# nlamprian/ICP

Measured on AMD Instinct MI355X. Metric: ICP iterations/sec at |F|=|M|=16384, |R|=256, higher is better.
Workload: dtype f32

## Files before the change

### icp_amd/csrc/icp_capi.hip

```cpp
#include "icp_host.h"

using namespace icp_host;

namespace {

void free_all (icp_context *h)
{
    drop_graphs (h);
    for (void *q : h->dev_allocs) (void) hipFree (q);
    h->dev_allocs.clear ();
    if (h->hF) (void) hipHostFree (h->hF);
    if (h->hM) (void) hipHostFree (h->hM);
    if (h->hT) (void) hipHostFree (h->hT);
    if (h->hState) (void) hipHostFree (h->hState);
    if (h->hMirror) (void) hipHostFree (h->hMirror);
    if (h->hTrackMirror) (void) hipHostFree (h->hTrackMirror);
    h->hState = nullptr; h->hMirror = h->hTrackMirror = nullptr; h->hstate_fresh = false;
    h->run = run_ctl {}; h->track_k_hist[0] = h->track_k_hist[1] = 0; h->track_hist_frame = 0;
    if (h->dCloud) (void) hipFree (h->dCloud);
    if (h->dCloudOut) (void) hipFree (h->dCloudOut);
    h->hF = h->hM = h->hT = nullptr; h->dCloud = h->dCloudOut = nullptr; h->cloud_cap = 0;
    h->dF = h->dM = nullptr; h->ownF = h->ownM = true;
    for (int k = 0; k < 2; ++k) {
        if (h->hBand[k]) (void) hipHostFree (h->hBand[k]);
// ... 132 lines not shown
    if (h->stream2) (void) hipStreamDestroy (h->stream2);
    if (h->stream) (void) hipStreamDestroy (h->stream);
    delete h;
    return ICP_OK;
}
ICP_CATCH_ALL

static int write_color_kappa (icp_context *h)
{
    uint32_t bits; std::memcpy (&bits, &h->color_kappa, sizeof bits);
    HIPCHK (h, hipMemsetD32Async (reinterpret_cast<hipDeviceptr_t> (icp_color_kappa (h->p)), (int) bits, 1, h->stream));
    return ICP_OK;
}

static int write_robust_scale (icp_context *h)
{
    uint32_t bits; std::memcpy (&bits, &h->robust_scale, sizeof bits);
    HIPCHK (h, hipMemsetD32Async (reinterpret_cast<hipDeviceptr_t> (icp_robust_scale (h->p)), (int) bits, 1, h->stream));
    return ICP_OK;
}

int icp_init_batched (icp_handle h, uint32_t batch, uint32_t m, uint32_t nr, float a, float c,
                      uint32_t max_iterations, double angle_threshold, double translation_threshold) try
{
    api_guard guard_ (h);
    if (!h) return ICP_EINVAL;
    if (m == 0) return fail (h, ICP_EINVAL, "The sets of landmarks cannot have zero points");
    if (nr == 0) return fail (h, ICP_EINVAL, "The sets of representatives cannot have zero points");
    if (a == 0.f) return fail (h, ICP_EINVAL, "The alpha parameter cannot be equal to zero");
    if (m % 2) return fail (h, ICP_EINVAL, "The number of points in the array must be a multiple of 2");
    if (batch == 0 || batch > 65535u) return fail (h, ICP_EINVAL, "batch must be in [1, 65535]");
    if (max_iterations == 0) return fail (h, ICP_EINVAL, "max_iterations must be positive");
    uint32_t nrx, nry, side;
    if (!reps_grid (m, nr, &nrx, &nry, &side))
        return fail (h, ICP_EINVAL, "nr must be a power of two whose grid tiles the sqrt(m) x sqrt(m) landmark grid");
    if (nr > 32768u) return fail (h, ICP_EINVAL, "nr must be <= 32768");
    if (m > (1u << 20)) return fail (h, ICP_EINVAL, "m must be <= 2^20");
    int rc = set_device (h); if (rc) return rc;
    if ((rc = run_close_all (h))) return rc;
    if (h->copy_stream) HIPCHK (h, hipStreamSynchronize (h->copy_stream));
    if (h->stream2) HIPCHK (h, hipStreamSynchronize (h->stream2));
    if (h->stream) HIPCHK (h, hipStreamSynchronize (h->stream));
    int rot = h->p.rot, weighted = h->p.weighted, pmode = h->p.power_mode, fused = h->p.fused, chain = h->p.chain;
    const float dist_scale = h->p.dist_scale;
    const uint32_t reject = h->p.reject; const float reject_d2 = h->p.reject_d2, reject_max_dist = h->p.reject_max_dist, trim_keep = h->p.trim_keep;
    const uint32_t metric = h->p.metric, nrm_grid = h->p.nrm_grid; const float p2pl_mu = h->p.p2pl_mu;
    free_all (h);
    icp_params &p = h->p;
    p = icp_params {};
    p.rot = rot; p.weighted = weighted; p.power_mode = pmode; p.check = 0; p.fused = fused; p.chain = chain; p.emit = 1;
    p.dist_scale = dist_scale;
    p.reject = reject; p.reject_d2 = reject_d2; p.reject_max_dist = reject_max_dist; p.trim_keep = trim_keep;
    p.metric = metric; p.nrm_grid = nrm_grid; p.p2pl_mu = p2pl_mu;
    p.m = m; p.nr = nr; p.batch = batch; p.side = side; p.nrx = nrx; p.nry = nry;
    p.a = a; p.c = c;
    {
        auto magic = [] (uint32_t d) { return d > 1u ? (uint32_t) ((1ull << 32) / d + 1ull) : 0u; };
        p.side_magic = magic (side); p.cellw_magic = magic (side / nrx); p.cellh_magic = magic (side / nry);
    }
    h->max_iterations = max_iterations; h->angle_threshold = angle_threshold; h->translation_threshold = translation_threshold;
    p.tan_half_thr = std::tan (angle_threshold * M_PI / 360.0);
    p.trans_thr = translation_threshold;
    p.nwg = (m + 127u) / 128u;
    p.nwp = p.nwg; if (p.nwp != 1 && (p.nwp % 4)) p.nwp += 4 - p.nwp % 4;
    uint32_t n4 = m; if (n4 % 4) n4 += 4 - n4 % 4;
    p.G = n4 / 4;
    p.nsp = (p.G + 511u) / 512u; if (p.nsp != 1 && (p.nsp % 4)) p.nsp += 4 - p.nsp % 4;
    p.nchunk = (m + ICP_CHUNK - 1) / ICP_CHUNK;
    p.nb = (m + 63u) / 64u;
    { const uint32_t ng = (p.nb + 127u) / 128u; p.ng_magic = ng > 1u ? (uint32_t) ((1ull << 32) / ng + 1ull) : 0u; }

    const size_t B = batch;
    float *F = nullptr, *M = nullptr;
    if ((rc = dalloc (h, &F, B * m * 8))) return rc;
    if ((rc = dalloc (h, &M, B * m * 8))) return rc;
    h->dF = F; h->dM = M; p.F = F; p.M = M; h->lm[0] = F; h->lm[1] = M;
    if ((rc = dalloc (h, &p.R, B * nr * 8))) return rc;
    p.n16 = (nr + 15u) / 16u;
    p.nb = (m + 63u) / 64u;
    p.tbox = icp_tbox_of (p); p.n1k = (nr + p.tbox - 1u) / p.tbox;
    p.s2wave = icp_s2_wave_of (p);
    { const char *e = std::getenv ("ICP_AMD_XCDMAP"); p.xcdmap = e ? (e[0] == '1') : (B == 1u); }
    { const char *e = std::getenv ("ICP_AMD_WARM_SEED"); p.warm_seed = (e && e[0] == '1') ? 1u : 0u; }
    p.gtile = 0u;
    if (nrx % 4u == 0u && nry % 4u == 0u && !std::getenv ("ICP_AMD_STRIP_GROUPS")) { uint32_t lg = 0; while ((4u << lg) < nrx) ++lg; p.gtile = lg + 1u; }
    if ((rc = dalloc (h, &p.GB, B * 2 * (p.n16 + p.n1k)))) return rc;
    if ((rc = dalloc (h, &p.XP, icp_xp_layout_of (batch, m).total))) return rc;
    if ((rc = dalloc (h, &p.XQ, B * m * 8))) return rc;
    if ((rc = dalloc (h, &p.OL, B * ICP_OL_STRIDE (nr)))) return rc;
    p.nlb = m / 16u + 2u;
    if ((rc = dalloc (h, &p.LB, B * 3 * p.nlb))) return rc;
    if ((rc = dalloc (h, &p.rep_src, B * nr))) return rc;
    if ((rc = dalloc (h, &p.owner, B * m))) return rc;
    if ((rc = dalloc (h, &p.N, 2 * B * nr))) return rc;
    if ((rc = dalloc (h, &p.O, B * nr))) return rc;
    if ((rc = dalloc (h, &p.perm, B * m))) return rc;
    if ((rc = dalloc (h, &p.chunk_hist, B * p.nchunk * nr))) return rc;
    if ((rc = dalloc (h, &p.blist, B * p.nb * 64))) return rc;
    if ((rc = dalloc (h, &p.bn, B * p.nb))) return rc;
    if ((rc = dalloc (h, &p.brank, B * m))) return rc;
    if ((rc = dalloc (h, &p.rid, B * m))) return rc;
    if ((rc = dalloc (h, &p.nn_id, B * m))) return rc;
    if ((rc = dalloc (h, &p.PF, B * m))) return rc;
    if ((rc = dalloc (h, &p.PM, B * m))) return rc;
    if ((rc = dalloc (h, &p.wpart, B * 2 * p.nwp))) return rc;
    if ((rc = dalloc (h, &p.mpart, B * 2 * p.nwg))) return rc;
    if ((rc = dalloc (h, &p.mscr, B * 2 * ((p.nwg + 127u) / 128u)))) return rc;
    if ((rc = dalloc (h, &p.spart, B * 11 * p.nsp * 8))) return rc;
    if ((rc = dalloc (h, &p.mom, icp_mom_layout_of (batch, m, p.nb).total))) return rc;
    if ((rc = write_color_kappa (h))) return rc;
    if ((rc = write_robust_scale (h))) return rc;
    if ((rc = dalloc (h, &p.ml1, B * 18 * ((p.nb + 127u) / 128u)))) return rc;
    if ((rc = dalloc (h, &p.cst, B * 2))) return rc;
    if ((rc = dalloc (h, &p.st, B))) return rc;
    if ((rc = dalloc (h, &p.st_prev, B))) return rc;
    if (!h->dTin) HIPCHK (h, hipMalloc ((void **) &h->dTin, 8 * sizeof (float)));
    HIPCHK (h, hipHostMalloc ((void **) &h->hF, B * m * 8 * sizeof (float), hipHostMallocDefault));
    HIPCHK (h, hipHostMalloc ((void **) &h->hM, B * m * 8 * sizeof (float), hipHostMallocDefault));
    HIPCHK (h, hipHostMalloc ((void **) &h->hT, 64 * sizeof (float), hipHostMallocDefault));
    HIPCHK (h, hipHostMalloc ((void **) &h->hState, B * sizeof (icp_reg_state), hipHostMallocMapped | hipHostMallocCoherent));
    HIPCHK (h, hipHostMalloc ((void **) &h->hMirror, B * sizeof (unsigned long long), hipHostMallocMapped | hipHostMallocCoherent));
    std::memset (h->hMirror, 0, B * sizeof (unsigned long long));
    icp_launch_reset_state (p, h->stream, 1);
    HIPCHK (h, hipGetLastError ());
    HIPCHK (h, hipStreamSynchronize (h->stream));
    h->inited = true; h->built = false;
    return ICP_OK;
}
ICP_CATCH_ALL

int icp_init (icp_handle h, uint32_t m, uint32_t nr, float a, float c, uint32_t max_iterations,
              double angle_threshold, double translation_threshold) try
{
    api_guard guard_ (h);
    return icp_init_batched (h, 1, m, nr, a, c, max_iterations, angle_threshold, translation_threshold);
}
ICP_CATCH_ALL

int icp_write_b (icp_handle h, uint32_t b, int mem, const void *host_ptr, int block) try
{
    api_guard guard_ (h);
    int rc = need (h, false); if (rc) return rc;
    if (b >= h->p.batch) return fail (h, ICP_EINVAL, "batch index out of range");
    if ((rc = set_device (h))) return rc;
    const size_t fm = (size_t) h->p.m * 8 * sizeof (float);
    switch (mem) {
        case ICP_MEM_F:
        case ICP_MEM_M: {
            float *stage = (mem == ICP_MEM_F ? h->hF : h->hM) + (size_t) b * h->p.m * 8;
            float *dst = (mem == ICP_MEM_F ? h->dF : h->dM) + (size_t) b * h->p.m * 8;
            hipEvent_t ev = h->evStage[mem == ICP_MEM_F ? 0 : 1];
            note_inputs_change (h);
            HIPCHK (h, hipEventSynchronize (ev));
            if (host_ptr) std::memcpy (stage, host_ptr, fm);
            HIPCHK (h, hipMemcpyAsync (dst, stage, fm, hipMemcpyHostToDevice, h->stream));
            HIPCHK (h, hipEventRecord (ev, h->stream));
            break;
        }
        case ICP_MEM_T: {
            HIPCHK (h, hipEventSynchronize (h->evStage[2]));
            if (host_ptr) std::memcpy (h->hT, host_ptr, 8 * sizeof (float));
            HIPCHK (h, hipMemcpyAsync (h->dTin, h->hT, 8 * sizeof (float), hipMemcpyHostToDevice, h->stream));
            HIPCHK (h, hipEventRecord (h->evStage[2], h->stream));
            { const long long kb = h->k_base; note_enqueue (h); h->k_base = kb; }
            icp_launch_set_T (h->p, b, h->dTin, h->stream);
            HIPCHK (h, hipGetLastError ());
// ... 860 lines not shown
```

### icp_amd/csrc/icp_search.h

```cpp
#pragma once
#include "icp_kernels.h"

static __device__ __forceinline__ float sum4 (float4 v) { return ((v.x + v.y) + v.z) + v.w; }
static __device__ __forceinline__ uint32_t ks_hole_bit (float4 mg) { return (mg.x == 0.f && mg.y == 0.f && mg.z == 0.f) ? 0x80000000u : 0u; }

#define KS_SPLIT LPQ
#define KS_QPW (64 / KS_SPLIT)
#define KS_TILE 1024u
#ifndef ICP_S2_DEPTH16
#define ICP_S2_DEPTH16 8u
#endif
#ifndef ICP_S2_UNCOND
#define ICP_S2_UNCOND 128u
#endif
#ifndef ICP_S1_ORIGIN_LIST
#define ICP_S1_ORIGIN_LIST 1
#endif
#ifndef ICP_OL_STAGED_MIN
#define ICP_OL_STAGED_MIN 32u
#endif
#ifndef ICP_S1_SEED
#define ICP_S1_SEED 1
#endif
#ifndef ICP_S1_REJECT_MIN_NR
// ... 562 lines not shown
    unsigned long long k4[4], k2[2], k1;
#pragma unroll
    for (int j = 0; j < 4; ++j) {
        const bool odd = (lane & 1u) != 0u;
        const unsigned long long keep = odd ? key[2 * j + 1] : key[2 * j], send = odd ? key[2 * j] : key[2 * j + 1];
        k4[j] = min64 (keep, xchg_dpp (send, std::integral_constant<int, 0xB1> {}));
    }
#pragma unroll
    for (int j = 0; j < 2; ++j) {
        const bool odd = (lane & 2u) != 0u;
        const unsigned long long keep = odd ? k4[2 * j + 1] : k4[2 * j], send = odd ? k4[2 * j] : k4[2 * j + 1];
        k2[j] = min64 (keep, xchg_dpp (send, std::integral_constant<int, 0x4E> {}));
    }
    {
        const bool odd = (lane & 4u) != 0u;
        const unsigned long long keep = odd ? k2[1] : k2[0], send = odd ? k2[0] : k2[1];
        k1 = min64 (keep, xchg_lane (send, lane ^ 4u));
    }
    k1 = min64 (k1, xchg_lane (k1, lane ^ 8u));
    k1 = min64 (k1, xchg_lane (k1, lane ^ 16u));
    k1 = min64 (k1, xchg_lane (k1, lane ^ 32u));
    k1 = xchg_lane (k1, (lane & 56u) | (lane >> 3));
    dmin = __uint_as_float ((uint32_t) (k1 >> 32)); jmin = (uint32_t) k1;
    {
        uint32_t nl = (je - o + 7u) >> 3;
        nl = max (nl, (uint32_t) __builtin_amdgcn_update_dpp (0, (int) nl, 0x140, 0xF, 0xF, true));
        nl = max (nl, (uint32_t) __builtin_amdgcn_update_dpp ((int) nl, (int) nl, 0x142, 0xA, 0xF, false));
        nl = max (nl, (uint32_t) __builtin_amdgcn_update_dpp ((int) nl, (int) nl, 0x143, 0xC, 0xF, false));
        const uint32_t ntrips = (uint32_t) __builtin_amdgcn_readlane ((int) nl, 63);
        if (__builtin_expect (ntrips > ICP_S2W_UNCOND / 8u, 0)) {
            const uint32_t ss = lane & 7u;
            float best2 = dmin; uint32_t bj = 0xFFFFFFFFu;
            const float4 a4 = s_qa[qe], c4 = s_qc[qe];
            ks_list_tail<8> (XQb, o, je, (max (je, 1u) - 1u) << 5, ICP_S2W_UNCOND / 16u, ntrips, a4.x, a4.y, a4.z, c4.x, c4.y, c4.z, alpha, dr, b, lane, ss, best2, bj);
            const uint32_t pos = bj != 0xFFFFFFFFu ? min (o + ss + bj * 8u, max (je, 1u) - 1u) : jmin;
            const float d2 = ks_grp_min_f<8> (best2);
            jmin = ks_grp_min_u<8> (best2 == d2 ? pos : 0xFFFFFFFFu);
            dmin = d2;
        }
    }
}

template <int LPQ>
static __device__ __forceinline__ void ks_stage2_lanes (const char *XQb, uint32_t o, uint32_t n, bool valid, float qx, float qy, float qz, float qr, float qg, float qb,
                                                        float alpha, float dr, uint32_t b, uint32_t lane, uint32_t ss, float &dmin, uint32_t &jmin)
{
    float best2 = __builtin_inff (); uint32_t bj = 0xFFFFFFFFu;
    const float2v vq_xr = { qx, qr }, vq_yg = { qy, qg }, vq_zb = { qz, qb };
    {
        constexpr uint32_t KS_DEPTH = (KS_SPLIT == 16) ? ICP_S2_DEPTH16 : 4u;
        const uint32_t je = valid ? o + n : o;
        uint32_t nl = (je - o + KS_SPLIT - 1u) / KS_SPLIT;
        if (KS_SPLIT == 8) nl = max (nl, (uint32_t) __builtin_amdgcn_update_dpp (0, (int) nl, 0x140, 0xF, 0xF, true));
        nl = max (nl, (uint32_t) __builtin_amdgcn_update_dpp ((int) nl, (int) nl, 0x142, 0xA, 0xF, false));
        nl = max (nl, (uint32_t) __builtin_amdgcn_update_dpp ((int) nl, (int) nl, 0x143, 0xC, 0xF, false));
        const uint32_t ntrips = (uint32_t) __builtin_amdgcn_readlane ((int) nl, 63);
        const uint32_t alast = (max (je, 1u) - 1u) << 5;
        constexpr uint32_t KS_UNC = ICP_S2_UNCOND / KS_SPLIT;
        const uint32_t ntr0 = (ICP_S2_UNCOND == 0u || ntrips <= 2u * KS_UNC) ? ntrips : KS_UNC;
        for (uint32_t tb = 0; tb < ntr0; tb += KS_DEPTH) {
            const uint32_t a0 = (o + ss + tb * KS_SPLIT) << 5, nt = min (KS_DEPTH, ntr0 - tb);
            float4 g[KS_DEPTH], c[KS_DEPTH];
#pragma unroll
            for (uint32_t t = 0; t < KS_DEPTH; ++t) {
                if (t >= nt) break;
                const char *rec = XQb + min (a0 + t * (KS_SPLIT * 32u), alast);
                g[t] = *reinterpret_cast<const float4 *> (rec); c[t] = *reinterpret_cast<const float4 *> (rec + 16);
            }
#pragma unroll
            for (uint32_t t = 0; t < KS_DEPTH; ++t) {
                if (t >= nt) break;
                KS_CAND (g[t], c[t], tb + t);
            }
        }
        if (__builtin_expect (ntrips > ntr0, 0))
            ks_list_tail<LPQ> (XQb, o, je, alast, ICP_S2_UNCOND / 16u, ntrips, qx, qy, qz, qr, qg, qb, alpha, dr, b, lane, ss, best2, bj);
        if (bj != 0xFFFFFFFFu) bj = min (o + ss + bj * KS_SPLIT, max (je, 1u) - 1u);
        if (je == o) { best2 = __builtin_inff (); bj = 0xFFFFFFFFu; }
    }
    dmin = ks_grp_min_f<KS_SPLIT> (best2);
    jmin = ks_grp_min_u<KS_SPLIT> (best2 == dmin ? bj : 0xFFFFFFFFu);
}

template <bool FUSED, bool CHAIN, int MINW, int LPQ, bool OWNER, bool PRUNE, bool REJ>
static __device__ __forceinline__ void ks_epilogue (const icp_params &p, float4 *s_qa, uint4 *s_qb, const float4 *s_qc, const uint32_t *s_slot, double (*s_mom)[64], float *s_w, const float4 *R4, const char *XQb,
                                                    uint32_t b, uint32_t m, uint32_t nr, uint32_t check_flags, uint32_t tid, uint32_t lane, uint32_t slice, uint32_t tile_id,
                                                    uint32_t qe, uint32_t ss, uint32_t i, bool valid, uint32_t o, uint32_t n, uint32_t rstar, float dr, float dmin, uint32_t jmin,
                                                    float qx, float qy, float qz)
{
    if (ss == 0u) {
        const bool empty = (n == 0u);
        s_qa[qe] = make_float4 (qx, qy, qz, empty ? dr : dmin);
        s_qb[qe] = make_uint4 (empty ? rstar : ((jmin == 0xFFFFFFFFu) ? o : jmin), rstar, (valid ? 1u : 0u) | (empty ? 2u : 0u), i);
    }
    __syncthreads ();
    if (slice == 0u) {
        const float4 qa = s_qa[lane]; const uint4 qb = s_qb[lane];
        const uint32_t eo = (PRUNE && ICP_S1_ORIGIN_LIST) ? s_slot[lane] : lane;
        const bool v = (qb.z & 1u) != 0u, empty = (qb.z & 2u) != 0u;
        const float ex = qa.x, ey = qa.y, ez = qa.z, d = p.dist_scale * qa.w;
        const uint32_t ei = qb.w;
        float w = 0.f, f0 = 0.f, f1 = 0.f, f2 = 0.f;
        bool acc = v;
        if (v) {
            uint32_t id;
            if (empty) {
                const float4 nn = R4[2 * (size_t) qb.x];
                const uint32_t *rsrc = p.rep_src;
                if constexpr (MINW == 4) {
                    typedef uint32_t __attribute__ ((address_space (1))) *gu32;
                    rsrc = (const uint32_t *) (gu32) ks_params_from_kernarg ()->rep_src;
                }
                id = rsrc[(size_t) b * nr + qb.x]; f0 = nn.x; f1 = nn.y; f2 = nn.z;
            } else {
                const char *rec = XQb + (qb.x << 5);
                const float4 wg = *reinterpret_cast<const float4 *> (rec), wc = *reinterpret_cast<const float4 *> (rec + 16);
                f0 = wg.x; f1 = wg.z; f2 = wc.x; id = __float_as_uint (wc.z);
            }
            w = p.weighted ? 100.f / (100.f + d) : 1.f;
            if constexpr (REJ) {
                bool rej = false;
                if (p.reject & 1u)
                    rej = (__float_as_uint (s_qc[lane].w) >> 31) != 0u || (f0 == 0.f && f1 == 0.f && f2 == 0.f);
                if (p.reject & ICP_REJECT_DIST_ON) {
                    const float gx = ex - f0, gy = ey - f1, gz = ez - f2;
                    rej = rej || !(((gx * gx + gy * gy) + gz * gz) <= p.reject_d2);
                }
                if (rej) { w = 0.f; acc = false; }
            }
            icp_dist_id di; di.dist = d; di.id = id;
            const icp_params *pe = &p;
            if constexpr (MINW == 2 && !OWNER) {
                            pe = ks_params_from_kernarg ();
            }
            typedef char __attribute__ ((address_space (1))) *gchar;
            char *o_nn = (char *) (gchar) reinterpret_cast<char *> (pe->nn_id + (size_t) b * m), *o_pf = (char *) (gchar) reinterpret_cast<char *> (pe->PF + (size_t) b * m);
            char *o_pm = (char *) (gchar) reinterpret_cast<char *> (pe->PM + (size_t) b * m), *o_rid = (char *) (gchar) reinterpret_cast<char *> (pe->rid + (size_t) b * m);
            const bool emit = !FUSED || (check_flags & 8u);
            if (emit) {
                *reinterpret_cast<icp_dist_id *> (o_nn + (ei << 3)) = di;
                *reinterpret_cast<float4 *> (o_pf + (ei << 4)) = make_float4 (f0, f1, f2, w);
                *reinterpret_cast<float4 *> (o_pm + (ei << 4)) = make_float4 (ex, ey, ez, d);
            }
            if (emit || PRUNE) *reinterpret_cast<uint32_t *> (o_rid + (ei << 2)) = qb.y;
        }
        if constexpr (FUSED) {
            double W = (double) w;
            double g0 = acc ? (double) f0 : 0.0, g1 = acc ? (double) f1 : 0.0, g2 = acc ? (double) f2 : 0.0;
            double q0 = (double) ex, q1 = (double) ey, q2 = (double) ez;
            if (!acc) { W = 0.0; q0 = q1 = q2 = 0.0; }
            double wq0 = W * q0, wq1 = W * q1, wq2 = W * q2;
            s_mom[0][eo] = W;
            s_mom[1][eo] = W * g0; s_mom[2][eo] = W * g1; s_mom[3][eo] = W * g2;
            s_mom[4][eo] = wq0; s_mom[5][eo] = wq1; s_mom[6][eo] = wq2;
            s_mom[7][eo] = wq0 * g0; s_mom[8][eo] = wq0 * g1; s_mom[9][eo] = wq0 * g2;
            s_mom[10][eo] = wq1 * g0; s_mom[11][eo] = wq1 * g1; s_mom[12][eo] = wq1 * g2;
            s_mom[13][eo] = wq2 * g0; s_mom[14][eo] = wq2 * g1; s_mom[15][eo] = wq2 * g2;
            s_mom[16][eo] = W * ((g0 * g0 + g1 * g1) + g2 * g2);
            s_mom[17][eo] = W * ((q0 * q0 + q1 * q1) + q2 * q2);
        } else
            s_w[eo] = w;
    }
    KS_STAMP (6)
    __syncthreads ();
    if constexpr (FUSED) {
        if (slice * 4u >= (uint32_t) ICP_NMOM) return;
        const uint32_t l = lane & 15u, mrow = slice * 4u + (lane >> 4);
        const uint32_t k = min (mrow, (uint32_t) ICP_NMOM - 1u);
        double c0 = s_mom[k][l] + s_mom[k][l + 32], c1 = s_mom[k][l + 16] + s_mom[k][l + 48];
        double v = row_tree_tail_d (c0 + c1);
        const uint32_t obuf = CHAIN ? (p.slot ^ 1u) : 0u;
        double *momw = p.mom;
        if constexpr (MINW == 4) {
            typedef double __attribute__ ((address_space (1))) *gf64;
            momw = (double *) (gf64) ks_params_from_kernarg ()->mom;
        }
        if (l == 0 && mrow < ICP_NMOM) momw[(((size_t) b * 2 + obuf) * ICP_NMOM + mrow) * p.nb + tile_id] = v;
    } else if (slice == 0 && (p.weighted || REJ)) {
        const uint32_t l = lane & 15u;
        float a[4] = { s_w[l], s_w[l + 16], s_w[l + 32], s_w[l + 48] };
        float v = row_tree4 (a);
        if (lane == 0) p.wpart[(size_t) b * 2 * p.nwp + blockIdx.x] = v;
    }
    KS_STAMP (7)
}

static __device__ __forceinline__ void ks_owner_lists_tail (const icp_params &p, uint4 *s_qb, uint32_t b, uint32_t m, uint32_t nb, uint32_t lane, uint32_t slice, uint32_t qe,
                                                            uint32_t ss, bool valid, uint32_t rstar)
{
    if (ss == 0u) s_qb[qe] = make_uint4 (rstar, valid ? 1u : 0u, 0u, 0u);
    __syncthreads ();
    if (slice != 0u) return;
    const uint4 e4 = s_qb[lane];
    const bool v = e4.y != 0u;
    const uint32_t own = v ? e4.x : 0xFFFFFFFFu, ip = blockIdx.x * 64u + lane;
    uint32_t rank = 0u, kk = 0u;
    uint2 *bl = p.blist + ((size_t) b * nb + blockIdx.x) * 64u;
    for (unsigned long long rem = __ballot (v); rem; ++kk) {
        const uint32_t o = (uint32_t) __builtin_amdgcn_readlane ((int) own, (int) __builtin_ctzll (rem));
        const unsigned long long same = __ballot (own == o);
        if (own == o) rank = (uint32_t) __builtin_popcountll (same & ((1ull << lane) - 1ull));
        if (lane == 0) bl[kk] = make_uint2 (o, (uint32_t) __builtin_popcountll (same));
        rem &= ~same;
    }
    if (lane == 0) p.bn[(size_t) b * nb + blockIdx.x] = kk;
    if (v) { p.owner[(size_t) b * m + ip] = own; p.brank[(size_t) b * m + ip] = (uint8_t) rank; }
    return;
}

template <int LPQ, int TILE>
static __device__ __forceinline__ uint32_t ks_coarse_pass (const float4 *s_box, uint32_t box0, float qx, float qy, float qz, uint32_t ss, uint32_t tn_, float lim_)
{
    const uint32_t ngt = (((tn_ + 1u) >> 1) + KS_SPLIT - 1u) / KS_SPLIT;
    uint32_t cm = 0u;
    auto test = [&] (uint32_t t, uint32_t g) {
        const float4 lo = s_box[box0 + 2 * g], hi = s_box[box0 + 2 * g + 1];
        const float ex = fmaxf (fmaxf (lo.x - qx, qx - hi.x), 0.f);
        const float ey = fmaxf (fmaxf (lo.y - qy, qy - hi.y), 0.f);
        const float ez = fmaxf (fmaxf (lo.z - qz, qz - hi.z), 0.f);
        const float bound = __builtin_fmaf (ez, ez, __builtin_fmaf (ey, ey, ex * ex));
        if (bound < lim_) cm |= 1u << t;
    };
    if constexpr (TILE == 256) {
#pragma unroll 1
        for (uint32_t t = 0, g = ss; g < ngt; ++t, g += KS_SPLIT) test (t, g);
    } else
        for (uint32_t t = 0, g = ss; g < ngt; ++t, g += KS_SPLIT) test (t, g);
    return cm;
}

template <int LPQ>
static __device__ __forceinline__ void ks_fine_pass (const float4 *s_pair, uint32_t pair0, float qx, float qy, float qz, float qr, float qg, float qb, float alpha,
                                                     uint32_t gt_lg1, uint32_t ss, uint32_t t0_, uint32_t npair_, uint32_t cmask_, float &best, uint32_t &bid)
{
    const uint32_t ngt_ = (npair_ + KS_SPLIT - 1u) / KS_SPLIT;
    const float2v vqx = { qx, qx }, vqy = { qy, qy }, vqz = { qz, qz }, vqr = { qr, qr }, vqg = { qg, qg }, vqb = { qb, qb };
    const float2v va = { alpha, alpha };
    for (uint32_t t = 0; t * KS_SPLIT < ngt_; ++t) {
        unsigned long long bal = __ballot ((cmask_ >> t) & 1u);
        if (bal == 0ull) continue;
        bal |= bal >> 32; bal |= bal >> 16;
        if (KS_SPLIT == 8) bal |= bal >> 8;
        uint32_t need = (uint32_t) bal & ((1u << KS_SPLIT) - 1u);
        while (need) {
            const uint32_t sg = (uint32_t) __builtin_ctz (need);
            need &= need - 1u;
            const uint32_t gl = sg + KS_SPLIT * t;
            const uint32_t P = (KS_SPLIT == 8 && gt_lg1) ? (((4u * (gl >> (gt_lg1 - 1u)) + (ss >> 1)) << gt_lg1) + 2u * (gl & ((1u << (gt_lg1 - 1u)) - 1u)) + (ss & 1u))
                                                          : gl * KS_SPLIT + ss;
            if (P < npair_) {
                const uint32_t P3 = pair0 + __umul24 (P, 3u);
                float4 A = s_pair[P3], B = s_pair[P3 + 1], C = s_pair[P3 + 2];
                float2v x = { A.x, A.y }, y = { A.z, A.w }, z = { B.x, B.y }, r = { B.z, B.w }, g = { C.x, C.y }, bb = { C.z, C.w };
                float2v dx = vqx - x, dy = vqy - y, dz = vqz - z, dr = vqr - r, dg = vqg - g, db = vqb - bb;
                float2v geo = __builtin_elementwise_fma (dz, dz, __builtin_elementwise_fma (dy, dy, dx * dx));
                float2v pho = __builtin_elementwise_fma (db, db, __builtin_elementwise_fma (dg, dg, dr * dr));
                float2v d = __builtin_elementwise_fma (va, pho, geo);
                const uint32_t r0 = t0_ + 2u * P;
                if (d.x < best) { best = d.x; bid = r0; }
                if (d.y < best) { best = d.y; bid = r0 + 1u; }
            }
        }
    }
}

template <bool FUSED, bool CHAIN, int MINW, int LPQ, bool OWNER = false, int ROT = 1, int TILE = 1024, bool SINGLE = false, bool S2W = false, bool HOSTRUN = false,
          bool REJ = false>
__global__ __launch_bounds__ (64 * LPQ, TILE == 256 ? 8 : MINW) void k_search (const float *gM, const float *gR, icp_reg_state *gst, const double *gmom,
                                                              uint32_t m, uint32_t nr, uint32_t side, uint32_t tpr_magic,
                                                              uint32_t nb, uint32_t check_flags, icp_params p)
{
    constexpr uint32_t KT = (uint32_t) TILE;
    constexpr bool MASKED = (TILE == 256) && !SINGLE && (MINW == 4);
    if constexpr (SINGLE) __builtin_assume (nr <= KT);
    if constexpr (MASKED) __builtin_assume (nr > KT && nr <= 32u * KT);
    const uint32_t b = blockIdx.y, check = check_flags & 1u;
    icp_reg_state *st = (CHAIN && !(check_flags & 2u)) ? gst + (size_t) b * 2 : gst + b;
#ifdef ICP_DBG_STAMPS
    { const uint32_t tid = threadIdx.x; unsigned long long t_; asm volatile ("s_memtime %0\n\ts_waitcnt lgkmcnt(0)" : "=s"(t_) :: "memory");
      KS_STAMP_STORE (8) }
#endif

    constexpr uint32_t NBUF = MASKED ? 2u : 1u, PB = 3u * KT / 2u, BB = 2u * (KT / 16u);
    __shared__ float4 s_pair[NBUF * PB];
    __shared__ uint2 s_on[(MASKED && OWNER) ? 1 : KT];
    __shared__ uint32_t s_tmask;
    __shared__ uint32_t s_ovote;
    __shared__ float4 s_box[NBUF * BB];
    __shared__ float4 s_tbox[(MINW == 4 && !SINGLE) ? 2 * 32 : 2];
    __shared__ float s_w[64];
    __shared__ float4 s_qc[64];
    __shared__ float4 s_qa[64];
    __shared__ uint4 s_qb[64];
    __shared__ uint32_t s_slot[(ICP_S1_SEED && ICP_S1_ORIGIN_LIST && MINW == 4) ? 64 : 1];
    __shared__ double s_mom[FUSED ? ICP_NMOM : 1][64];
    __shared__ icp_fin_result s_fin;
    __shared__ double s_l1[CHAIN ? ICP_NMOM : 1][CHAIN ? 32 : 1];
    __shared__ double s_t[ICP_NMOM];

    const uint32_t tid = threadIdx.x, lane = tid & 63u;
    const uint32_t slice = __builtin_amdgcn_readfirstlane (tid >> 6);
    const uint32_t qe = slice * KS_QPW + lane / KS_SPLIT, ss = lane & (KS_SPLIT - 1u);
    const bool qwave = CHAIN ? slice == 0u : slice == KS_SPLIT - 1u;
    constexpr bool OWNER_LISTS = OWNER && MINW == 2;
    const uint32_t tile_id = OWNER_LISTS ? blockIdx.x : (FUSED && (MINW == 2 || (check_flags & 64u))) ? ks_tile_of_block (blockIdx.x, nb) : blockIdx.x;
    const uint32_t iq = OWNER_LISTS ? blockIdx.x * 64u + lane :
                        FUSED ? fused_query_index (m, side, tpr_magic, tile_id, lane)
                              : (blockIdx.x >> 1) * 128u + 2u * lane + (blockIdx.x & 1u);

    const float4 *M4 = reinterpret_cast<const float4 *> (gM + (size_t) b * m * 8);
    const float4 *R4 = reinterpret_cast<const float4 *> (gR + (size_t) b * nr * 8);

    uint32_t sv = OWNER ? 0u : state_load_lanes (st);
    uint32_t run_over = 0u;
    if constexpr (CHAIN) {
        static_assert (ICP_ST_DW (T) == 0 && ICP_ST_DW (Tk) == 8 && ICP_ST_DW (R) == 16 && ICP_ST_DW (Rk) == 25 && ICP_ST_DW (reserved0) == 60, "state layout");
        if (check_flags & 16u) {
            constexpr unsigned long long ones = (1ull << 3) | (1ull << 7) | (1ull << 11) | (1ull << 15) | (1ull << 16) | (1ull << 20) | (1ull << 24) |
                                                (1ull << 25) | (1ull << 29) | (1ull << 33);
            if (lane < ICP_ST_DW (reserved0)) sv = ((ones >> lane) & 1ull) ? 0x3F800000u : 0u;
        }
    }
    double ma0[8];
    if constexpr (CHAIN) fused_moment_loads<64 * LPQ> (gmom + (size_t) b * 2 * ICP_NMOM * nb, nb, 0u, ma0);
    float *s_pairf = reinterpret_cast<float *> (s_pair);
    const uint32_t tn0 = min (KT, nr);
    float4 rg[2], rc[2]; uint2 ron[2];
    uint32_t ht = 0u, tnH = 0u;
#pragma unroll
    for (int u = 0; u < 2; ++u) {
        uint32_t k = tid + (uint32_t) u * 64u * KS_SPLIT;
        if (MASKED && u == 0) continue;
        rg[u] = make_float4 (0.f, 0.f, 0.f, 0.f); rc[u] = rg[u];
        if constexpr (OWNER_LISTS) {
            if (k < tn0) {
                const uint32_t src = rep_src_index (p, k);
                rg[u] = M4[2 * (size_t) src]; rc[u] = M4[2 * (size_t) src + 1];
                if (blockIdx.x == 0) {
                    float4 *Rw = reinterpret_cast<float4 *> (p.R + (size_t) b * nr * 8);
                    Rw[2 * (size_t) k] = rg[u]; Rw[2 * (size_t) k + 1] = rc[u];
                    p.rep_src[(size_t) b * nr + k] = src;
                }
            }
        } else if (!MASKED && k < tn0) { rg[u] = R4[2 * (size_t) k]; rc[u] = R4[2 * (size_t) k + 1]; }
    }
    const uint32_t ic = min (iq, m - 1u);
    typedef float ks_f4 __attribute__ ((ext_vector_type (4)));
    ks_f4 mgv = { 0.f, 0.f, 0.f, 1.f }, mcv = mgv;
    if (qwave) { mgv = *reinterpret_cast<const ks_f4 *> (M4 + 2 * (size_t) ic); mcv = *reinterpret_cast<const ks_f4 *> (M4 + 2 * (size_t) ic + 1); }
    if constexpr (MASKED) {
        const uint32_t i0 = (uint32_t) __builtin_amdgcn_readfirstlane ((int) min (FUSED ? fused_query_index (m, side, tpr_magic, tile_id, 0u) : (blockIdx.x >> 1) * 128u + (blockIdx.x & 1u), m - 1u));
        const uint32_t cell = p.side_magic ? cell_rep_of (p, i0) : 0u;
        ht = min (cell, nr - 1u) / KT; tnH = min (KT, nr - ht * KT);
        if (ICP_HOME_MODE != 3 && tid < tnH) { rg[0] = R4[2 * (size_t) (ht * KT + tid)]; rc[0] = R4[2 * (size_t) (ht * KT + tid) + 1]; }
    }
    const uint32_t *gO = p.O + (size_t) b * nr, *gN = p.N + (size_t) b * nr;
#pragma unroll
    for (int u = 0; u < 2; ++u) {
        uint32_t k = tid + (uint32_t) u * 64u * KS_SPLIT;
        ron[u] = make_uint2 (0u, 0u);
        if (!OWNER && !MASKED && k < tn0) ron[u] = make_uint2 (gO[k], gN[k]);
        if (!OWNER && MASKED && u == 0 && tid < tnH) ron[0] = make_uint2 (gO[ht * KT + tid], gN[ht * KT + tid]);
    }
    if constexpr (CHAIN && HOSTRUN) { if (p.run_flag) run_over = (p.run_flag[b] == p.epoch) ? 1u : 0u; }
    constexpr bool PRUNE = ICP_S1_SEED && MINW == 4;
    const bool prune = PRUNE && p.a > 0.f;
    const uint32_t gt_lg1 = p.gtile;
// ... 233 lines not shown
            float *dst = s_pairf + (tn >> 1) * 12u + 1u;
            const float qnan = __builtin_nanf ("");
            dst[0] = qnan; dst[2] = qnan; dst[4] = qnan; dst[6] = qnan; dst[8] = qnan; dst[10] = qnan;
        }
        if (!(CHAIN && handed && t0 == 0u && !(tn & 1u))) __syncthreads ();
        if (t0 == 0) {
            const float4 a4 = s_qa[qe], c4 = s_qc[qe];
            if constexpr (PRUNE && ICP_S1_ORIGIN_LIST) { if (prune) n_origin = (uint32_t) __builtin_amdgcn_readfirstlane ((int) __float_as_uint ((!SINGLE && nr > KT) ? s_tbox[1].w : s_box[1].w)); }
            qx = a4.x; qy = a4.y; qz = a4.z; i = __float_as_uint (a4.w); valid = i < m;
            qr = c4.x; qg = c4.y; qb = c4.z; seed = __float_as_uint (c4.w);
        }
        KS_STAMP (1)
        const uint32_t npair = (tn + 1u) >> 1;
        const float2v vqx = { qx, qx }, vqy = { qy, qy }, vqz = { qz, qz }, vqr = { qr, qr }, vqg = { qg, qg }, vqb = { qb, qb };
        const float2v va = { alpha, alpha };
        float lim = __builtin_inff ();
        if (t0 == 0 && prune) {
            const uint32_t sfl = seed >> 30;
            seed = min (seed & 0x3FFFFFFFu, nr - 1u);
            float sx, sy, sz, sr, sg, sb;
            if (MINW == 2 || nr <= KT) {
                const float *sp = s_pairf + (seed >> 1) * 12u + (seed & 1u);
                sx = sp[0]; sy = sp[2]; sz = sp[4]; sr = sp[6]; sg = sp[8]; sb = sp[10];
                asm volatile ("" : "+v"(sx), "+v"(sy), "+v"(sz), "+v"(sr), "+v"(sg), "+v"(sb));
            } else {
                const float4 g = R4[2 * (size_t) seed], c = R4[2 * (size_t) seed + 1];
                sx = g.x; sy = g.y; sz = g.z; sr = c.x; sg = c.y; sb = c.z;
            }
            if constexpr (ICP_S1_ORIGIN_LIST && MINW == 4)
                ks_seed_against_invalid (sfl, (!SINGLE && nr > KT) ? s_tbox + 1 : s_box + 1, nr, b, R4, seed, sx, sy, sz, sr, sg, sb);
            const float b0 = icp_metric8 (qx, qy, qz, qr, qg, qb, sx, sy, sz, sr, sg, sb, alpha);
            if (b0 >= 0.f && b0 < __builtin_inff ()) lim = __uint_as_float (__float_as_uint (b0) + 1u);
            s1_lim = lim;
        } else if (prune) lim = s1_lim;
        if (prune) {
            if (t0 == 0 && __ballot (tile_near (lim))) cmask = ks_coarse_pass<LPQ, TILE> (s_box, 0u, qx, qy, qz, ss, tn, lim);
            ks_fine_pass<LPQ> (s_pair, 0u, qx, qy, qz, qr, qg, qb, alpha, gt_lg1, ss, t0, npair, cmask, best, bid);
            s1_lim = fminf (lim, ks_grp_min_f<KS_SPLIT> (best));
        } else {
#pragma unroll 8
            for (uint32_t P = ss; P < npair; P += KS_SPLIT) {
                float4 A = s_pair[3 * P], B = s_pair[3 * P + 1], C = s_pair[3 * P + 2];
                float2v x = { A.x, A.y }, y = { A.z, A.w }, z = { B.x, B.y }, r = { B.z, B.w }, g = { C.x, C.y }, bb = { C.z, C.w };
                float2v dx = vqx - x, dy = vqy - y, dz = vqz - z, dr = vqr - r, dg = vqg - g, db = vqb - bb;
                float2v geo = __builtin_elementwise_fma (dz, dz, __builtin_elementwise_fma (dy, dy, dx * dx));
                float2v pho = __builtin_elementwise_fma (db, db, __builtin_elementwise_fma (dg, dg, dr * dr));
                float2v d = __builtin_elementwise_fma (va, pho, geo);
                const uint32_t r0 = t0 + 2u * P;
                if (d.x < best) { best = d.x; bid = r0; }
                if (d.y < best) { best = d.y; bid = r0 + 1u; }
            }
        }
    }
    KS_STAMP (14)
    if constexpr (PRUNE && ICP_S1_ORIGIN_LIST) {
        if (prune && __builtin_expect (n_origin != 0u, 0))
            ks_origin_section<KS_SPLIT, PB> (s_pair, &s_ovote, n_origin, nr, b, slice, tid, qx, qy, qz, qr, qg, qb, alpha, s1_lim, lane, ss, best, bid);
    }
    KS_KEEP (best, bid)
    KS_STAMP (2)
    const float dr = ks_grp_min_f<KS_SPLIT> (best);
    const bool named = PRUNE ? (best == dr && dr < __builtin_inff ()) : (best == dr);
    uint32_t rstar = ks_grp_min_u<KS_SPLIT> (named ? bid : 0xFFFFFFFFu);
    if (rstar == 0xFFFFFFFFu) rstar = 0u;
    if constexpr (OWNER_LISTS) {
        ks_owner_lists_tail (p, s_qb, b, m, nb, lane, slice, qe, ss, valid, rstar);
        return;
    } else if constexpr (OWNER) {
        if (ss == 0u && valid) p.owner[(size_t) b * m + i] = rstar;
        return;
    }
    KS_KEEP (dr, rstar)
    KS_STAMP (3)
    uint32_t o, n;
    if constexpr (MINW == 2) { const uint2 on = s_on[rstar]; o = on.x; n = on.y; }
    else if constexpr (MASKED) {
        if (rstar / KT == ht) { const uint2 on = s_on[rstar - ht * KT]; o = on.x; n = on.y; asm volatile ("" : "+v"(o), "+v"(n)); }
        else { o = gO[rstar]; n = gN[rstar]; }
    }
    else if (nr <= KT) { const uint2 on = s_on[rstar]; o = on.x; n = on.y; asm volatile ("" : "+v"(o), "+v"(n)); }
    else { o = gO[rstar]; n = gN[rstar]; }

    float dmin; uint32_t jmin;
    if constexpr (S2W) {
        static_assert (MINW == 4 && LPQ == 8 && !OWNER, "lanes = candidates: the dense search variants");
        ks_stage2_wave (XQb, o, n, valid, rstar, qx, qy, qz, qr, qg, qb, alpha, dr, b, lane, s_qa, s_qc, qe, dmin, jmin);
    } else ks_stage2_lanes<LPQ> (XQb, o, n, valid, qx, qy, qz, qr, qg, qb, alpha, dr, b, lane, ss, dmin, jmin);
    KS_KEEP (dmin, jmin)
    KS_STAMP (5)
    ks_epilogue<FUSED, CHAIN, MINW, LPQ, OWNER, PRUNE, REJ> (p, s_qa, s_qb, s_qc, s_slot, s_mom, s_w, R4, XQb, b, m, nr, check_flags, tid, lane, slice, tile_id, qe, ss, i, valid, o, n, rstar, dr, dmin, jmin,
                                                        qx, qy, qz);
}


static inline uint32_t icp_tpr_magic (uint32_t side)
{
    const uint32_t tpr = side >> 3;
    return tpr ? (uint32_t) ((1ull << 32) / tpr + 1ull) : 0u;
}
#define KS_FLAGS(p) ((uint32_t) ((p).check ? 1u : 0u) | ((p).emit ? 8u : 0u) | ((p).warm_seed ? 32u : 0u) | ((p).xcdmap ? 64u : 0u))
#define KS_ARGS p.M, p.R, p.st, (const double *) p.mom, p.m, p.nr, p.side, icp_tpr_magic (p.side), p.nb, KS_FLAGS (p), p
#define KS_CHAIN_ARGS p.M, p.R, p.cst + p.slot, (const double *) p.mom + (size_t) p.slot * ICP_NMOM * p.nb, p.m, p.nr, p.side, icp_tpr_magic (p.side), p.nb, KS_FLAGS (p), p

template <bool REJ>
void ks_launch_dense (const icp_params &p, hipStream_t s)
{
    const bool t256 = icp_dense_tile (p) == 256u, multi = p.nr > 256u;
    if (p.fused) {
        if (p.s2wave && multi && t256) hipLaunchKernelGGL ((k_search<true, false, 4, 8, false, 1, 256, false, true, false, REJ>), dim3 (p.nb, p.batch), dim3 (512), 0, s, KS_ARGS);
        else if (p.s2wave && t256) hipLaunchKernelGGL ((k_search<true, false, 4, 8, false, 1, 256, true, true, false, REJ>), dim3 (p.nb, p.batch), dim3 (512), 0, s, KS_ARGS);
        else if (p.s2wave) hipLaunchKernelGGL ((k_search<true, false, 4, 8, false, 1, 1024, false, true, false, REJ>), dim3 (p.nb, p.batch), dim3 (512), 0, s, KS_ARGS);
        else if (multi && t256) hipLaunchKernelGGL ((k_search<true, false, 4, 8, false, 1, 256, false, false, false, REJ>), dim3 (p.nb, p.batch), dim3 (512), 0, s, KS_ARGS);
        else if (t256) hipLaunchKernelGGL ((k_search<true, false, 4, 8, false, 1, 256, true, false, false, REJ>), dim3 (p.nb, p.batch), dim3 (512), 0, s, KS_ARGS);
        else hipLaunchKernelGGL ((k_search<true, false, 4, 8, false, 1, 1024, false, false, false, REJ>), dim3 (p.nb, p.batch), dim3 (512), 0, s, KS_ARGS);
    } else {
        if (p.s2wave && multi && t256) hipLaunchKernelGGL ((k_search<false, false, 4, 8, false, 1, 256, false, true, false, REJ>), dim3 (2 * p.nwg, p.batch), dim3 (512), 0, s, KS_ARGS);
        else if (p.s2wave && t256) hipLaunchKernelGGL ((k_search<false, false, 4, 8, false, 1, 256, true, true, false, REJ>), dim3 (2 * p.nwg, p.batch), dim3 (512), 0, s, KS_ARGS);
        else if (p.s2wave) hipLaunchKernelGGL ((k_search<false, false, 4, 8, false, 1, 1024, false, true, false, REJ>), dim3 (2 * p.nwg, p.batch), dim3 (512), 0, s, KS_ARGS);
        else if (multi && t256) hipLaunchKernelGGL ((k_search<false, false, 4, 8, false, 1, 256, false, false, false, REJ>), dim3 (2 * p.nwg, p.batch), dim3 (512), 0, s, KS_ARGS);
        else if (t256) hipLaunchKernelGGL ((k_search<false, false, 4, 8, false, 1, 256, true, false, false, REJ>), dim3 (2 * p.nwg, p.batch), dim3 (512), 0, s, KS_ARGS);
        else hipLaunchKernelGGL ((k_search<false, false, 4, 8, false, 1, 1024, false, false, false, REJ>), dim3 (2 * p.nwg, p.batch), dim3 (512), 0, s, KS_ARGS);
    }
}

template <bool REJ>
void ks_launch_latency (const icp_params &p, hipStream_t s)
{
    if (p.fused) hipLaunchKernelGGL ((k_search<true, false, 2, 16, false, 1, 1024, false, false, false, REJ>), dim3 (p.nb, p.batch), dim3 (1024), 0, s, KS_ARGS);
    else hipLaunchKernelGGL ((k_search<false, false, 2, 16, false, 1, 1024, false, false, false, REJ>), dim3 (2 * p.nwg, p.batch), dim3 (1024), 0, s, KS_ARGS);
}

template <bool REJ>
void ks_launch_chain_one (const icp_params &p0, hipStream_t s, uint32_t j, bool fresh, bool emit)
{
    icp_params p = p0;
    p.slot = j & 1u;
    p.emit = emit ? 1 : 0;
    const uint32_t first_flags = 2u | (fresh ? 16u : 0u);
#define KS_CHAIN_LAUNCH(ROT_, HR_)                                                                                                              \
    do {                                                                                                                                        \
        if (j == 0) hipLaunchKernelGGL ((k_search<true, true, 2, 16, false, ROT_, 1024, false, false, HR_, REJ>), dim3 (p.nb, p.batch), dim3 (1024), 0, s, p.M, p.R, p.st, \
                                        (const double *) p.mom, p.m, p.nr, p.side, icp_tpr_magic (p.side), p.nb, KS_FLAGS (p) | first_flags, p);     \
        else hipLaunchKernelGGL ((k_search<true, true, 2, 16, false, ROT_, 1024, false, false, HR_, REJ>), dim3 (p.nb, p.batch), dim3 (1024), 0, s, KS_CHAIN_ARGS);     \
    } while (0)
    const bool hostrun = p.hmirror != nullptr;
    if (p.rot == 1) { if (hostrun) KS_CHAIN_LAUNCH (1, true); else KS_CHAIN_LAUNCH (1, false); }
    else            { if (hostrun) KS_CHAIN_LAUNCH (0, true); else KS_CHAIN_LAUNCH (0, false); }
#undef KS_CHAIN_LAUNCH
}
```

Measured before the change: 114,100.

## Stage per-block candidate lists in shared memory for stage-2 search

For the MINW==2, LPQ==16 search variant, each block gathers the union of its queries' representative candidate lists into the reused s_pair LDS buffer, provided the total fits 1024 records and no list exceeds 256. Stage-2 nearest-neighbour scans and the epilogue's winner fetch then read from LDS instead of repeatedly loading global XQ records. This removes redundant global loads when several queries share a representative. The cost is an extra barrier, a wave-serial ballot loop to assign offsets, and a larger shared array. The path can be disabled with ICP_AMD_S2_SHARED=0.

```diff
diff --git a/icp_amd/csrc/icp_capi.hip b/icp_amd/csrc/icp_capi.hip
--- a/icp_amd/csrc/icp_capi.hip
+++ b/icp_amd/csrc/icp_capi.hip
@@ -238,6 +238,7 @@
     p.s2wave = icp_s2_wave_of (p);
     { const char *e = std::getenv ("ICP_AMD_XCDMAP"); p.xcdmap = e ? (e[0] == '1') : (B == 1u); }
     { const char *e = std::getenv ("ICP_AMD_WARM_SEED"); p.warm_seed = (e && e[0] == '1') ? 1u : 0u; }
+    { const char *e = std::getenv ("ICP_AMD_S2_SHARED"); if (e && e[0] == '0') p.warm_seed |= 2u; }
     p.gtile = 0u;
     if (nrx % 4u == 0u && nry % 4u == 0u && !std::getenv ("ICP_AMD_STRIP_GROUPS")) { uint32_t lg = 0; while ((4u << lg) < nrx) ++lg; p.gtile = lg + 1u; }
     if ((rc = dalloc (h, &p.GB, B * 2 * (p.n16 + p.n1k)))) return rc;
diff --git a/icp_amd/csrc/icp_search.h b/icp_amd/csrc/icp_search.h
--- a/icp_amd/csrc/icp_search.h
+++ b/icp_amd/csrc/icp_search.h
@@ -668,15 +668,56 @@
     jmin = ks_grp_min_u<KS_SPLIT> (best2 == dmin ? bj : 0xFFFFFFFFu);
 }
 
+#define KS_STAGE_RECS 1024u
+#define KS_STAGE_HEAD 256u
+static __device__ __forceinline__ void ks_stage2_staged (const float4 *rec, uint32_t loff, uint32_t o, uint32_t n, bool valid, float qx, float qy, float qz, float qr, float qg,
+                                                         float qb, float alpha, uint32_t ss, float &dmin, uint32_t &jmin)
+{
+    static_assert (KS_STAGE_HEAD == 2u * ICP_S2_UNCOND || ICP_S2_UNCOND == 0u, "a staged block's lists are those ks_stage2_lanes scans without chunk tests");
+    float best2 = __builtin_inff (); uint32_t bj = 0xFFFFFFFFu;
+    const float2v vq_xr = { qx, qr }, vq_yg = { qy, qg }, vq_zb = { qz, qb };
+    constexpr uint32_t KS_DEPTH = ICP_S2_DEPTH16;
+    const uint32_t nq = valid ? n : 0u;
+    uint32_t nl = (nq + 15u) / 16u;
+    nl = max (nl, (uint32_t) __builtin_amdgcn_update_dpp ((int) nl, (int) nl, 0x142, 0xA, 0xF, false));
+    nl = max (nl, (uint32_t) __builtin_amdgcn_update_dpp ((int) nl, (int) nl, 0x143, 0xC, 0xF, false));
+    const uint32_t ntrips = (uint32_t) __builtin_amdgcn_readlane ((int) nl, 63);
+    const uint32_t plast = max (nq, 1u) - 1u;
+    for (uint32_t tb = 0; tb < ntrips; tb += KS_DEPTH) {
+        const uint32_t nt = min (KS_DEPTH, ntrips - tb);
+        float4 g[KS_DEPTH], c[KS_DEPTH];
+#pragma unroll
+        for (uint32_t t = 0; t < KS_DEPTH; ++t) {
+            if (t >= nt) break;
+            const uint32_t k = loff + min (ss + (tb + t) * 16u, plast);
+            g[t] = rec[k]; c[t] = rec[KS_STAGE_RECS + k];
+        }
+#pragma unroll
+        for (uint32_t t = 0; t < KS_DEPTH; ++t) {
+            if (t >= nt) break;
+            KS_CAND (g[t], c[t], tb + t);
+        }
+    }
+    if (bj != 0xFFFFFFFFu) bj = o + min (ss + bj * 16u, plast);
+    if (nq == 0u) { best2 = __builtin_inff (); bj = 0xFFFFFFFFu; }
+    dmin = ks_grp_min_f<16> (best2);
+    jmin = ks_grp_min_u<16> (best2 == dmin ? bj : 0xFFFFFFFFu);
+}
+
 template <bool FUSED, bool CHAIN, int MINW, int LPQ, bool OWNER, bool PRUNE, bool REJ>
 static __device__ __forceinline__ void ks_epilogue (const icp_params &p, float4 *s_qa, uint4 *s_qb, const float4 *s_qc, const uint32_t *s_slot, double (*s_mom)[64], float *s_w, const float4 *R4, const char *XQb,
                                                     uint32_t b, uint32_t m, uint32_t nr, uint32_t check_flags, uint32_t tid, uint32_t lane, uint32_t slice, uint32_t tile_id,
                                                     uint32_t qe, uint32_t ss, uint32_t i, bool valid, uint32_t o, uint32_t n, uint32_t rstar, float dr, float dmin, uint32_t jmin,
-                                                    float qx, float qy, float qz)
-{
+                                                    float qx, float qy, float qz, const float4 *lrec = nullptr, uint32_t loff = 0u)
+{
+    constexpr bool STAGED = MINW == 2 && LPQ == 16 && !OWNER;
     if (ss == 0u) {
         const bool empty = (n == 0u);
         s_qa[qe] = make_float4 (qx, qy, qz, empty ? dr : dmin);
+        if constexpr (STAGED) {
+            const uint32_t jw = (jmin == 0xFFFFFFFFu) ? o : jmin;
+            s_qb[qe] = make_uint4 (empty ? rstar : jw, rstar, (valid ? 1u : 0u) | (empty ? 2u : 0u) | ((lrec && !empty) ? (loff + (jw - o)) << 2 : 0u), i);
+        } else
         s_qb[qe] = make_uint4 (empty ? rstar : ((jmin == 0xFFFFFFFFu) ? o : jmin), rstar, (valid ? 1u : 0u) | (empty ? 2u : 0u), i);
     }
     __syncthreads ();
@@ -699,9 +740,19 @@
                 }
                 id = rsrc[(size_t) b * nr + qb.x]; f0 = nn.x; f1 = nn.y; f2 = nn.z;
             } else {
-                const char *rec = XQb + (qb.x << 5);
-                const float4 wg = *reinterpret_cast<const float4 *> (rec), wc = *reinterpret_cast<const float4 *> (rec + 16);
-                f0 = wg.x; f1 = wg.z; f2 = wc.x; id = __float_as_uint (wc.z);
+                auto from_global = [&] () {
+                    const char *rec = XQb + (qb.x << 5);
+                    const float4 wg = *reinterpret_cast<const float4 *> (rec), wc = *reinterpret_cast<const float4 *> (rec + 16);
+                    f0 = wg.x; f1 = wg.z; f2 = wc.x; id = __float_as_uint (wc.z);
+                };
+                if constexpr (STAGED) {
+                    if (lrec) {
+                        const uint32_t k = min (qb.z >> 2, KS_STAGE_RECS - 1u);
+                        const float4 wg = lrec[k], wc = lrec[KS_STAGE_RECS + k];
+                        f0 = wg.x; f1 = wg.z; f2 = wc.x; id = __float_as_uint (wc.z);
+                        asm volatile ("" : "+v"(f0), "+v"(f1), "+v"(f2), "+v"(id));
+                    } else from_global ();
+                } else from_global ();
             }
             w = p.weighted ? 100.f / (100.f + d) : 1.f;
             if constexpr (REJ) {
@@ -868,7 +919,10 @@
 #endif
 
     constexpr uint32_t NBUF = MASKED ? 2u : 1u, PB = 3u * KT / 2u, BB = 2u * (KT / 16u);
-    __shared__ float4 s_pair[NBUF * PB];
+    constexpr bool STAGED = MINW == 2 && LPQ == 16 && !OWNER;
+    static_assert (!STAGED || (NBUF * PB <= 2u * KS_STAGE_RECS && KT == 1024u), "the staged lists reuse the representatives' tile buffer");
+    __shared__ float4 s_pair[STAGED ? 2u * KS_STAGE_RECS : NBUF * PB];
+    __shared__ uint32_t s_rs[STAGED ? 64 : 1];
     __shared__ uint2 s_on[(MASKED && OWNER) ? 1 : KT];
     __shared__ uint32_t s_tmask;
     __shared__ uint32_t s_ovote;
@@ -1268,14 +1322,49 @@
     else { o = gO[rstar]; n = gN[rstar]; }
 
     float dmin; uint32_t jmin;
-    if constexpr (S2W) {
+    const float4 *lrec = nullptr; uint32_t loff = 0u;
+    if constexpr (STAGED) {
+        if (!(check_flags & 128u)) {
+            if (ss == 0u) s_rs[qe] = valid ? rstar : 0xFFFFFFFFu;
+            __syncthreads ();
+            const uint32_t rl = s_rs[lane];
+            uint2 onl = make_uint2 (0u, 0u);
+            if (rl != 0xFFFFFFFFu) onl = s_on[rl];
+            const bool has = rl != 0xFFFFFFFFu && onl.y != 0u;
+            uint32_t tot = 0u, lofl = 0u, src = 0u, longest = 0u; bool live = false;
+            for (unsigned long long rem = __ballot (has); rem; ) {
+                const int l0 = (int) __builtin_ctzll (rem);
+                const uint32_t ru = (uint32_t) __builtin_amdgcn_readlane ((int) rl, l0), ou = (uint32_t) __builtin_amdgcn_readlane ((int) onl.x, l0),
+                               nu = (uint32_t) __builtin_amdgcn_readlane ((int) onl.y, l0);
+                if (rl == ru) lofl = tot;
+                if (tid >= tot) { src = ou + (tid - tot); live = tid - tot < nu; }
+                longest = max (longest, nu);
+                tot += (nu + 15u) & ~15u;
+                rem &= ~__ballot (rl == ru);
+            }
+            KS_STAMP (15)
+            if (tot <= KS_STAGE_RECS && longest <= KS_STAGE_HEAD) {
+                if (live) {
+                    const char *rec = XQb + (src << 5);
+                    const float4 g = *reinterpret_cast<const float4 *> (rec), c = *reinterpret_cast<const float4 *> (rec + 16);
+                    s_pair[tid] = g; s_pair[KS_STAGE_RECS + tid] = c;
+                }
+                loff = (uint32_t) __builtin_amdgcn_ds_bpermute ((int) (qe << 2), (int) lofl);
+                __syncthreads ();
+                lrec = s_pair;
+            }
+            KS_STAMP (4)
+        }
+        if (lrec) ks_stage2_staged (lrec, loff, o, n, valid, qx, qy, qz, qr, qg, qb, alpha, ss, dmin, jmin);
+        else ks_stage2_lanes<LPQ> (XQb, o, n, valid, qx, qy, qz, qr, qg, qb, alpha, dr, b, lane, ss, dmin, jmin);
+    } else if constexpr (S2W) {
         static_assert (MINW == 4 && LPQ == 8 && !OWNER, "lanes = candidates: the dense search variants");
         ks_stage2_wave (XQb, o, n, valid, rstar, qx, qy, qz, qr, qg, qb, alpha, dr, b, lane, s_qa, s_qc, qe, dmin, jmin);
     } else ks_stage2_lanes<LPQ> (XQb, o, n, valid, qx, qy, qz, qr, qg, qb, alpha, dr, b, lane, ss, dmin, jmin);
     KS_KEEP (dmin, jmin)
     KS_STAMP (5)
     ks_epilogue<FUSED, CHAIN, MINW, LPQ, OWNER, PRUNE, REJ> (p, s_qa, s_qb, s_qc, s_slot, s_mom, s_w, R4, XQb, b, m, nr, check_flags, tid, lane, slice, tile_id, qe, ss, i, valid, o, n, rstar, dr, dmin, jmin,
-                                                        qx, qy, qz);
+                                                        qx, qy, qz, lrec, loff);
 }
 
 
@@ -1284,7 +1373,7 @@
     const uint32_t tpr = side >> 3;
     return tpr ? (uint32_t) ((1ull << 32) / tpr + 1ull) : 0u;
 }
-#define KS_FLAGS(p) ((uint32_t) ((p).check ? 1u : 0u) | ((p).emit ? 8u : 0u) | ((p).warm_seed ? 32u : 0u) | ((p).xcdmap ? 64u : 0u))
+#define KS_FLAGS(p) ((uint32_t) ((p).check ? 1u : 0u) | ((p).emit ? 8u : 0u) | (((p).warm_seed & 1u) ? 32u : 0u) | ((p).xcdmap ? 64u : 0u) | (((p).warm_seed & 2u) ? 128u : 0u))
 #define KS_ARGS p.M, p.R, p.st, (const double *) p.mom, p.m, p.nr, p.side, icp_tpr_magic (p.side), p.nb, KS_FLAGS (p), p
 #define KS_CHAIN_ARGS p.M, p.R, p.cst + p.slot, (const double *) p.mom + (size_t) p.slot * ICP_NMOM * p.nb, p.m, p.nr, p.side, icp_tpr_magic (p.side), p.nb, KS_FLAGS (p), p
 
```

Measured after the change: 100,300, median of 2. 0.879x the previous value.
